# zhiyuns/REHRSeg

Measured on AMD Instinct MI355X. Metric: 3D patches/sec (fwd+bwd, 128^3 fp32), higher is better.
Workload: dtype f32; 1 GPU; FLAVR UNet_3D_3D(1,'unet_18',128,4) fwd+bwd+Adam, 1x1x128^3 patch per GPU, random-init weights; patches_per_gpu=1, global_batch=1, parallelism=dp1 (patch-parallel, flat-bucket RCCL all-reduce), wgrad_stream=True

## Files before the change

include/rehrseg_hip.h:

```cpp
#ifndef REHRSEG_HIP_H
#define REHRSEG_HIP_H

#include <stdint.h>

#ifdef __cplusplus
extern "C" {
#endif

#define REHR_OK 0
#define REHR_EINVAL -1
#define REHR_ENOSUP -2
#define REHR_EHIP -3

#define REHR_ACT_NONE 0
#define REHR_ACT_RELU 1
#define REHR_ACT_LRELU 2

typedef struct {
  int32_t count, off0, offs, k0, ks;
} rehr_axis_taps;

typedef struct {
  const float* x1;
  const float* x2;
// ... 3 lines not shown
  int32_t sd, sh, sw, bd, bh, bw;
  rehr_axis_taps td, th, tw;
  int32_t KH, KW;
  const float* wp;
  int32_t Npad;
  float* y;
  int32_t Dy, Hy, Wy, Cout, ldy;
  int32_t osd, osh, osw, obd, obh, obw;
  const float* bias;
  int32_t act;
  float slope;
  double* stats;
  int32_t stats_mode;
  int32_t tile_d, tile_h, tile_w;
  float* wino_ws;
  int64_t wino_ws_bytes;
  int32_t flags;
  int32_t debug_flags;
} rehr_gather_gemm_desc;

#define REHR_GG_Y_F32 1
#define REHR_GG_WS_READY 2
#define REHR_GG_WS_ONLY 4

#define REHR_DBG_GG_NO_HALO 1
#define REHR_DBG_GG_NO_FLAT8 2
#define REHR_DBG_GG_FLAT8_HALF 4
#define REHR_DBG_GG_FLAT8_FULL 8
#define REHR_DBG_GG_W32P_TWO_PER_CU 16
#define REHR_DBG_GG_W32P_ONE_PER_CU 32
#define REHR_DBG_GG_INTERLEAVE 64
#define REHR_DBG_GG_NO_TCONV_KS 128
#define REHR_DBG_GG_SLICE_MAJOR 256

int64_t rehr_gather_gemm_wino_bytes(const rehr_gather_gemm_desc* d);
#define REHR_GG_ROUTE_NONE 0
#define REHR_GG_ROUTE_FLAT8 1
#define REHR_GG_ROUTE_W32P 2
#define REHR_GG_ROUTE_BIG8 3
#define REHR_GG_ROUTE_SMALL 4
#define REHR_GG_ROUTE_FLAT22 5
#define REHR_GG_ROUTE_REGION22 6
int rehr_gather_gemm_wino_route(const rehr_gather_gemm_desc* d);
#define REHR_GG_DIRECT_NONE 0
#define REHR_GG_DIRECT_GENERIC 1
#define REHR_GG_DIRECT_HALO 2
#define REHR_GG_DIRECT_TCONV_KS 3
int rehr_gather_gemm_direct_route(const rehr_gather_gemm_desc* descs, int32_t count, int32_t bf16, int32_t* routes);
int rehr_gather_gemm_f32(const rehr_gather_gemm_desc* d, void* stream);
int rehr_gather_gemm_multi_f32(const rehr_gather_gemm_desc* descs, int32_t count,
                               void* stream);
int rehr_gather_gemm_wino_forms_f32(const rehr_gather_gemm_desc* descs, int32_t count, const float* w, int32_t D0,
                                    int32_t D1, int32_t T, int32_t dest_dim, int32_t dest_lo, int32_t src_lo,
                                    void* stream);
int rehr_gather_gemm_bf16(const rehr_gather_gemm_desc* d, void* stream);
int rehr_gather_gemm_multi_bf16(const rehr_gather_gemm_desc* descs, int32_t count, void* stream);
int rehr_pack_weights_bf16(const float* in, void* out, int32_t A, int32_t Apad, int32_t B, int32_t T,
                           int32_t transpose_ab, void* stream);

int rehr_sum_slabs_bias_act_f32(const float* slabs, int32_t S, int64_t slab_stride,
                                const float* bias, float* y, int64_t rows, int32_t C,
                                int32_t act, float slope, void* stream);

int rehr_sum_slabs_stats_f32(const float* slabs, int32_t S, int64_t slab_stride, const float* bias,
                             float* y, int32_t N, int64_t SV, int32_t C, int32_t act, float slope,
                             double* stats, void* stream);

int rehr_sum_slabs_bias_act_bf16(const float* slabs, int32_t S, int64_t slab_stride, const float* bias, void* y,
                                 int64_t rows, int32_t C, int32_t act, float slope, void* stream);
int rehr_sum_slabs_stats_bf16(const float* slabs, int32_t S, int64_t slab_stride, const float* bias, void* y,
                              int32_t N, int64_t SV, int32_t C, int32_t act, float slope, double* stats,
                              void* stream);

typedef struct {
  const float* l;
  int32_t ldl, Ca;
// ... 357 lines not shown
```

rehrseg_amd/csrc/gather_gemm.hip:

```cpp
#include "common.h"
#include "halo_shared.h"
#include "wino_shared.h"

namespace {

constexpr int BK = 32;
constexpr int LDS_LD = 36;
constexpr int NTHREADS = 256;

template <int BM, int BN, int WGM, int WGN, int LDSBUF>
__device__ __forceinline__ void gather_gemm_body(const GGParams& p, const int nblocks, const int logical_in = -1) {
  constexpr int WTM = BM / WGM, WTN = BN / WGN;
  constexpr int FM = WTM / 32, FN = WTN / 32;
  constexpr int AROWS = BM / 32, BROWS = BN / 32;
  static_assert(WGM * WGN == 4, "4 waves");
  const rehr_gather_gemm_desc& d = p.d;

  extern __shared__ __attribute__((aligned(16))) float smem[];
  float* As = smem;
  float* Bs = smem + LDSBUF * BM * LDS_LD;
  int* row_out = (int*)(Bs + LDSBUF * BN * LDS_LD);

  const int tid = threadIdx.x;
  const int lane = tid & 63, wave = tid >> 6;
// ... 382 lines not shown
    const rehr_axis_taps* ax[3] = {&d.td, &d.th, &d.tw};
    const int ext[3] = {T / (d.KH * d.KW), d.KH, d.KW};
    for (int a = 0; a < 3; ++a) {
      const int64_t first = ax[a]->k0, last = (int64_t)ax[a]->k0 + (int64_t)ax[a]->ks * (ax[a]->count - 1);
      if (first < 0 || first >= ext[a] || last < 0 || last >= ext[a]) return REHR_EINVAL;
    }
  }
  if (route[0].kind == DIRECT_TCONV_KS) return REHR_ENOSUP;
  WinoRoute r[MAX_PHASES];
  WinoPlan plan{};
  const WinoRoute joint = wino_joint_route(descs, count, plan);
  for (int i = 0; i < count; ++i) {
    r[i] = joint ? joint : wino_part_route(descs[i], count, plan);
    if (r[i] == WINO_NONE) return REHR_ENOSUP;
  }
  WinoWeightSrc src;
  const int64_t s0 = (int64_t)D1 * T, s1 = T;
  src.sn = dest_dim == 0 ? s0 : s1;
  src.sc = dest_dim == 0 ? s1 : s0;
  src.w = w + dest_lo * src.sn + src_lo * src.sc;
  return wino_forms_launch(r, descs, count, src, (hipStream_t)stream);
}

extern "C" int64_t rehr_gather_gemm_wino_bytes(const rehr_gather_gemm_desc* dp) {
  WinoPlan plan{};
  if (dp == nullptr || validate(*dp) != REHR_OK || wino_route(*dp, plan) == WINO_NONE) return 0;
  return plan.bytes;
}

extern "C" int rehr_gather_gemm_wino_route(const rehr_gather_gemm_desc* dp) {
  WinoPlan plan{};
  if (dp == nullptr || validate(*dp) != REHR_OK) return REHR_GG_ROUTE_NONE;
  const WinoRoute r = wino_route(*dp, plan);
  return r == WINO_NONE ? REHR_GG_ROUTE_NONE : (int)r | (plan.variant << 8);
}

extern "C" int rehr_gather_gemm_direct_route(const rehr_gather_gemm_desc* descs, int32_t count, int32_t bf16,
                                             int32_t* routes) {
  DirectRoute route[MAX_PHASES];
  if (routes == nullptr) return REHR_EINVAL;
  const int rc = direct_route(descs, count, bf16 ? 2 : 4, route);
  if (rc != REHR_OK) return rc;
  for (int i = 0; i < count; ++i) routes[i] = route[i].kind | (route[i].variant << 8);
  return REHR_OK;
}

extern "C" int rehr_gather_gemm_f32(const rehr_gather_gemm_desc* dp, void* stream) {
  if (dp == nullptr) return REHR_EINVAL;
  return rehr_gather_gemm_multi_f32(dp, 1, stream);
}
```

rehrseg_amd/csrc/wino_conv.hip:

```cpp
#include "common.h"
#include "wino_shared.h"
#include <cstdlib>

namespace {

constexpr int TH = 4, TW = 8;
constexpr int PH = 2 * TH + 2, PW = 2 * TW + 2;
constexpr int PVOX = PH * PW;
constexpr int LDX = 36;
constexpr int NX = (PVOX * 8 + 255) / 256;

struct WinoParams {
  rehr_gather_gemm_desc d;
  int nb_h, nb_w;
  int band_major;
  int kchunks;
  int dh0, dw0;
  const float* up;
  uint32_t up_bytes;
  int nsplit;
  rehr_axis_taps s_td[8];
  const float* s_up[8];
  uint32_t s_up_bytes[8];
  float* s_y[8];
// ... 188 lines not shown
#pragma unroll
    for (int q = 0; q < 16; ++q) t[rr][q] = ex[((rr * 2 + co) * 16 + q) * 64 + lane];
#pragma unroll
  for (int q = 0; q < 16; ++q) {
    const float yv = k0 * t[0][q] + t[1][q] + k2 * t[2][q] + k3 * t[3][q] + bv;
    const float v = fmaxf(yv, 0.f) + neg_slope * fminf(yv, 0.f);
    const int tile = (q & 3) + 8 * (q >> 2) + 4 * half;
    const int oh = oh0 + 2 * (tile / TW) + ro, ow = ow0 + 2 * (tile % TW) + co;
    const bool ok = colok & (oh < d.Lh) & (ow < d.Lw);
    if (ok) d.y[((((int64_t)n_img * d.Dy + od) * d.Hy + oh) * d.Wy + ow) * d.ldy + col_n] = v;
    s1_ += ok ? v : 0.f;
    s2_ += ok ? v * v : 0.f;
  }
  if (d.stats_mode != 0) {
    s1_ += __shfl_xor(s1_, 32, 64);
    s2_ += __shfl_xor(s2_, 32, 64);
    __syncthreads();
    float* red = smem;
    if (half == 0) {
      red[(r * 2 + 0) * 32 + col] = s1_;
      red[(r * 2 + 1) * 32 + col] = s2_;
    }
    __syncthreads();
    if (r == 0 && half == 0 && colok) {
      const float a1 = red[col] + red[64 + col] + red[128 + col] + red[192 + col];
      const float a2 = red[32 + col] + red[96 + col] + red[160 + col] + red[224 + col];
      double* st = d.stats + ((int64_t)n_img * d.Cout + col_n) * 2;
      atomicAdd(st, (double)a1);
      if (d.stats_mode == 2) atomicAdd(st + 1, (double)a2);
    }
  }
}

constexpr int PW2 = 18, PVOX2 = 18 * 18;
constexpr int RP2 = PW2 * LDX + 8;
constexpr int BUF2 = PW2 * RP2;

__global__ void wino_weights_frag_kernel(const rehr_gather_gemm_desc d, float* __restrict__ up, int kchunks) {
  const int cpad = kchunks * 32;
  const int64_t per = (int64_t)d.Npad * cpad;
  const int64_t per_src = (int64_t)d.Npad * d.Cin;
  const int64_t total = (int64_t)d.td.count * per;
  const int NT = d.Npad / 32;
  for (int64_t i = (int64_t)blockIdx.x * blockDim.x + threadIdx.x; i < total; i += (int64_t)gridDim.x * blockDim.x) {
    const int jd = (int)(i / per);
    const int64_t rem = i - (int64_t)jd * per;
    const int n = (int)(rem / cpad), ci = (int)(rem - (int64_t)n * cpad);
    float g[3][3];
#pragma unroll
    for (int jh = 0; jh < 3; ++jh)
#pragma unroll
      for (int jw = 0; jw < 3; ++jw) {
        const int a = d.bh + d.th.off0 + d.th.offs * jh + 1;
        const int b = d.bw + d.tw.off0 + d.tw.offs * jw + 1;
        const int wt = ((d.td.k0 + d.td.ks * jd) * d.KH + (d.th.k0 + d.th.ks * jh)) * d.KW + (d.tw.k0 + d.tw.ks * jw);
        const float v = ci < d.Cin ? d.wp[(int64_t)wt * per_src + (int64_t)n * d.Cin + ci] : 0.f;
#pragma unroll
        for (int aa = 0; aa < 3; ++aa)
#pragma unroll
          for (int bb = 0; bb < 3; ++bb)
            if (aa == a && bb == b) g[aa][bb] = v;
      }
    float u[16];
    wino_u33(g, u);
    const int nt = n >> 5, col = n & 31, chunk = ci >> 5, kk = (ci >> 3) & 3, half = (ci >> 2) & 1, e = ci & 3;
#pragma unroll
    for (int xi = 0; xi < 16; ++xi) {
      const int64_t o = (((((int64_t)jd * 16 + xi) * NT + nt) * kchunks + chunk) * 4 + kk) * 256 + (half * 32 + col) * 4 + e;
      up[o] = u[xi];
    }
  }
}

constexpr int NX8 = (PVOX2 * 8 + 511) / 512;

__global__ __launch_bounds__(512) void wino_conv_big8_kernel(const WinoParams p) {
  const rehr_gather_gemm_desc& d = p.d;
  extern __shared__ __attribute__((aligned(16))) float smem[];
  float* Xs = smem;
  constexpr int BUF = BUF2;

  const int tid = threadIdx.x, lane = tid & 63;
  const int wv = __builtin_amdgcn_readfirstlane(tid >> 6);
  const int r = wv & 3, fm = wv >> 2;
  const int half = lane >> 5, col = lane & 31;
  const int part = (p.nsplit > 1) ? (int)(blockIdx.z % p.nsplit) : 0;
  const int n_img = (p.nsplit > 1) ? (int)(blockIdx.z / p.nsplit) : (int)blockIdx.z;
  const rehr_axis_taps td = (p.nsplit > 1) ? p.s_td[part] : p.d.td;
  const float* const up = (p.nsplit > 1) ? p.s_up[part] : p.up;
  const uint32_t up_bytes = (p.nsplit > 1) ? p.s_up_bytes[part] : p.up_bytes;
  float* const yout = (p.nsplit > 1) ? p.s_y[part] : p.d.y;
  const int nt0 = blockIdx.y * 2, n0 = blockIdx.y * 64;
  int b = xcd_remap(blockIdx.x, gridDim.x);
  const int bw_ = b % p.nb_w; b /= p.nb_w;
  const int bh_ = p.band_major ? b / p.d.Ld : b % p.nb_h;
  const int od = p.band_major ? b % p.d.Ld : b / p.nb_h;
  const int oh0 = bh_ * 16, ow0 = bw_ * 16;

  const int i1 = (r == 0) ? 0 : 1, i2 = (r == 3) ? 3 : 2;
  const float s2 = (r == 1) ? 1.f : -1.f;
  const float rsign = (r == 2) ? -1.f : 1.f;
  const int th_ = fm * 4 + (col >> 3), tw_ = col & 7;
  const float* xa = Xs + (2 * th_ + i1) * RP2 + tw_ * LDX + 4 * half;
  const float* xb = Xs + (2 * th_ + i2) * RP2 + tw_ * LDX + 4 * half;

  int pvx[NX8];
  uint32_t pok = 0;
#pragma unroll
  for (int i = 0; i < NX8; ++i) {
    const int piece = tid + 512 * i;
    const int v = piece >> 3;
    const int ph = v / PW2, slot = v - ph * PW2;
    const int pw_ = slot < 9 ? 2 * slot : 2 * (slot - 9) + 1;
    const int ih = oh0 + p.dh0 + ph, iw = ow0 + p.dw0 + pw_;
    const bool ok = (piece < PVOX2 * 8) & ((unsigned)ih < (unsigned)d.Hi) & ((unsigned)iw < (unsigned)d.Wi);
    pvx[i] = ok ? ih * d.Wi + iw : 0;
    pok |= (ok ? 1u : 0u) << i;
  }
  const int pq = tid & 7;
  const uint32_t img_elems = (uint32_t)d.Di * d.Hi * d.Wi;
  constexpr int NXH = NX8 / 2;
  f32x4 rx[NXH];
  int jd_lo = td.count, jd_hi = -1;
  for (int j = 0; j < td.count; ++j) {
    const int id = od + d.bd + td.off0 + td.offs * j;
    if ((unsigned)id < (unsigned)d.Di) { jd_lo = min(jd_lo, j); jd_hi = max(jd_hi, j); }
  }
  const int items = p.kchunks * max(0, jd_hi - jd_lo + 1);
  struct Item { int chunk, jd; };
  auto advance = [&](Item& t) {
    if (++t.jd > jd_hi) { t.jd = jd_lo; ++t.chunk; }
  };
  auto fetch_to = [&](f32x4 (&rx)[NXH], const Item& t, const int lo) {
    const bool live = (t.chunk < p.kchunks) & (items > 0);
    const int jd = t.jd;
    const int cc = (live ? t.chunk : 0) * 32;
    const int id = od + d.bd + td.off0 + td.offs * jd;
    const bool first = cc < d.c1;
    const float* src = first ? d.x1 : d.x2;
    const uint32_t ld = (uint32_t)(first ? d.ldx1 : d.ldx2);
    const int coff = first ? cc : cc - d.c1;
    const uint32_t nrec = img_elems * ld * 4u;
    const __amdgpu_buffer_rsrc_t rs = __builtin_amdgcn_make_buffer_rsrc(
        const_cast<float*>(src) + (int64_t)n_img * img_elems * ld, 0, nrec, 0x00020000);
    const bool dok = live & ((unsigned)id < (unsigned)d.Di) & ((cc + pq * 4) < d.Cin);
    const uint32_t base = (uint32_t)(id * d.Hi * d.Wi) * ld * 4u + (uint32_t)(coff + pq * 4) * 4u;
#pragma unroll
    for (int i = 0; i < NXH; ++i) {
      const bool ok = dok & ((pok >> (lo + i)) & 1u);
      const uint32_t off = base + (uint32_t)pvx[lo + i] * ld * 4u;
      rx[i] = __builtin_bit_cast(f32x4, __builtin_amdgcn_raw_buffer_load_b128(rs, ok ? off : nrec, 0, 0));
    }
  };
  auto stage_from = [&](const f32x4 (&rx)[NXH], int buf, const int lo) {
#pragma unroll
    for (int i = 0; i < NXH; ++i) {
      const int piece = tid + 512 * (lo + i);
      const int v = piece >> 3, row = (v * 3641) >> 16;
      if (piece < PVOX2 * 8) *reinterpret_cast<f32x4*>(Xs + buf + v * LDX + row * 8 + pq * 4) = rx[i];
    }
  };
  auto fetch = [&](const Item& t, const int lo) { fetch_to(rx, t, lo); };
  auto stage = [&](int buf, const int lo) { stage_from(rx, buf, lo); };

  const __amdgpu_buffer_rsrc_t rsu =
      __builtin_amdgcn_make_buffer_rsrc(const_cast<float*>(up), 0, up_bytes, 0x00020000);
  const int NT = d.Npad / 32;
  const uint32_t xi_stride = (uint32_t)NT * p.kchunks * 4096u, nt_stride = (uint32_t)p.kchunks * 4096u;
  const uint32_t ulane = (uint32_t)lane * 16u;
  const uint32_t ubase = (uint32_t)(r * 4) * xi_stride + (uint32_t)nt0 * nt_stride;
  auto load_u = [&](const Item& t, const int kk, const int fn, f32x4 (&ub)[4]) {
    const int chunk = t.chunk < p.kchunks ? t.chunk : 0;
    const uint32_t base = ubase + (uint32_t)(t.jd * 16) * xi_stride + (uint32_t)(chunk * 4 + kk) * 1024u + fn * nt_stride;
#pragma unroll
    for (int c = 0; c < 4; ++c)
      ub[c] = __builtin_bit_cast(f32x4, __builtin_amdgcn_raw_buffer_load_b128(rsu, ulane, base + c * xi_stride, 0));
  };

  f32x16 acc[2][4];
#pragma unroll
  for (int fn = 0; fn < 2; ++fn)
#pragma unroll
    for (int c = 0; c < 4; ++c)
#pragma unroll
      for (int q = 0; q < 16; ++q) acc[fn][c][q] = 0.f;

  f32x4 ra[4], rb[4];
  auto issue_reads = [&](int buf, const int kk) {
#pragma unroll
    for (int j = 0; j < 4; ++j) {
// ... 72 lines not shown
  for (int it = 0; it < items; ++it) {
    const int cur = (it & 1) * BUF, nxt = cur ^ BUF;
    advance(ni);
    BIG8_PRIO(2);
    BIG8_KGROUP(0, VA, VB, ci, 1, issue_reads(cur, 1), fetch(ni, 0), (void)0)
    BIG8_PRIO(1);
    BIG8_KGROUP(1, VB, VA, ci, 2, issue_reads(cur, 2), (void)0, stage(nxt, 0))
    BIG8_KGROUP(2, VA, VB, ci, 3, issue_reads(cur, 3), fetch(ni, NXH), (void)0)
    __builtin_amdgcn_sched_barrier(0);
    BIG8_PRIO(0);
    stage(nxt, NXH);
    mfmas(0, VB, u0);
    __builtin_amdgcn_sched_barrier(0);
    load_u(ni, 0, 0, u0);
#ifdef BIG8_STAMPS
    const long long sa_ = __builtin_readcyclecounter();
#endif
    __syncthreads();
#ifdef BIG8_STAMPS
    b8_bar += __builtin_readcyclecounter() - sa_;
#endif
    __builtin_amdgcn_sched_barrier(0);
    BIG8_PRIO(3);
    issue_reads(nxt, 0);
    mfmas(1, VB, u1);
    combine(VA);
    __builtin_amdgcn_sched_barrier(0);
    load_u(ni, 0, 1, u1);
    ci = ni;
  }
#undef BIG8_KGROUP
  BIG8_PRIO(0);
#ifdef BIG8_STAMPS
  if ((threadIdx.x & 63) == 0 && blockIdx.x == 777 && blockIdx.y == 0 && blockIdx.z == 0)
    printf("big8 wave %d items %d: loop %lld cycles, barrier waits %lld\n", (int)(threadIdx.x >> 6), items,
           (long long)(__builtin_readcyclecounter() - b8_t0), b8_bar);
#endif
  __syncthreads();

  float* ex = smem;
#pragma unroll
  for (int fn = 0; fn < 2; ++fn) {
    const f32x16 T0 = (acc[fn][0] + acc[fn][1] - acc[fn][2]) * rsign;
    const f32x16 T1 = (acc[fn][1] + acc[fn][2] - acc[fn][3]) * rsign;
    float* e0 = ex + (((fm * 2 + fn) * 4 + r) * 2) * 16 * 64 + lane;
#pragma unroll
    for (int q = 0; q < 16; ++q) {
      e0[q * 64] = T0[q];
      e0[(16 + q) * 64] = T1[q];
    }
  }
  __syncthreads();
  const int ro = r >> 1, co = r & 1;
  const float k0 = ro == 0 ? 1.f : 0.f, k2 = ro == 0 ? 1.f : -1.f, k3 = ro == 0 ? 0.f : -1.f;
  const float neg_slope = d.act == REHR_ACT_NONE ? 1.f : (d.act == REHR_ACT_RELU ? 0.f : d.slope);
  float ssum[2][2];
  float* ybase = yout + ((((int64_t)n_img * d.Dy + od) * d.Hy + (oh0 + ro)) * d.Wy + (ow0 + co + 8 * half)) * d.ldy +
                 n0 + col;
  const int64_t rowstep = 2 * (int64_t)d.Wy * d.ldy, colstep = 2 * (int64_t)d.ldy;
  const bool interior = (oh0 + 16 <= d.Lh) & (ow0 + 16 <= d.Lw) & (n0 + 64 <= d.Cout);
#pragma unroll
  for (int fn = 0; fn < 2; ++fn) {
    const int col_n = n0 + fn * 32 + col;
    const bool colok = col_n < d.Cout;
    const float bv = (d.bias != nullptr && colok) ? d.bias[col_n] : 0.f;
    float s1_ = 0.f, s2_ = 0.f;
    const float* e0 = ex + ((fm * 2 + fn) * 4 * 2 + co) * 16 * 64 + lane;
    float t[4][16];
#pragma unroll
    for (int rr = 0; rr < 4; ++rr)
#pragma unroll
      for (int q = 0; q < 16; ++q) t[rr][q] = e0[(rr * 32 + q) * 64];
    float v[16];
#pragma unroll
    for (int q = 0; q < 16; ++q) {
      const float yv = k0 * t[0][q] + t[1][q] + k2 * t[2][q] + k3 * t[3][q] + bv;
      v[q] = fmaxf(yv, 0.f) + neg_slope * fminf(yv, 0.f);
    }
    float* yb = ybase + fn * 32 + (fm * 4) * rowstep;
    if (interior) {
#pragma unroll
      for (int q = 0; q < 16; ++q) {
        yb[(q >> 2) * rowstep + (q & 3) * colstep] = v[q];
        s1_ += v[q];
        s2_ += v[q] * v[q];
      }
    } else {
#pragma unroll
      for (int q = 0; q < 16; ++q) {
        const int oh = oh0 + 2 * (fm * 4 + (q >> 2)) + ro, ow = ow0 + 2 * ((q & 3) + 4 * half) + co;
        const bool ok = colok & (oh < d.Lh) & (ow < d.Lw);
        if (ok) yb[(q >> 2) * rowstep + (q & 3) * colstep] = v[q];
        s1_ += ok ? v[q] : 0.f;
        s2_ += ok ? v[q] * v[q] : 0.f;
      }
    }
    ssum[fn][0] = s1_ + __shfl_xor(s1_, 32, 64);
    ssum[fn][1] = s2_ + __shfl_xor(s2_, 32, 64);
  }
  if (d.stats_mode != 0) {
    __syncthreads();
    float* red = smem;
    if (half == 0) {
#pragma unroll
      for (int fn = 0; fn < 2; ++fn) {
        red[((wv * 2 + fn) * 2 + 0) * 32 + col] = ssum[fn][0];
        red[((wv * 2 + fn) * 2 + 1) * 32 + col] = ssum[fn][1];
      }
    }
    __syncthreads();
    if (wv < 2 && half == 0) {
      const int fn = wv, col_n = n0 + fn * 32 + col;
      if (col_n < d.Cout) {
        float a1 = 0.f, a2 = 0.f;
#pragma unroll
        for (int w = 0; w < 8; ++w) {
          a1 += red[((w * 2 + fn) * 2 + 0) * 32 + col];
          a2 += red[((w * 2 + fn) * 2 + 1) * 32 + col];
        }
        double* st = d.stats + ((int64_t)n_img * d.Cout + col_n) * 2;
        atomicAdd(st, (double)a1);
        if (d.stats_mode == 2) atomicAdd(st + 1, (double)a2);
      }
    }
  }
}

constexpr int W3_LD = 20, W3_RP = PW2 * W3_LD + 8;
template <int NFM> struct W3 {
  static constexpr int ROWS = 8 * NFM + 2, BUF = ROWS * W3_RP, VOX = ROWS * PW2, NTHR = 256 * NFM;
  static constexpr int NXT = (VOX * 4 + NTHR - 1) / NTHR;
};

template <int G>
__global__ __launch_bounds__(256 * G, G == 1 ? 2 : 1) void wino_conv_w32p_kernel(const WinoParams p) {
  constexpr int NTHR = 256 * G, VOX = W3<2 * G>::VOX, BUF = W3<2 * G>::BUF + 32;
  constexpr int W3P_NX = (VOX * 4 + NTHR - 1) / NTHR;
  const rehr_gather_gemm_desc& d = p.d;
  extern __shared__ __attribute__((aligned(16))) float smem[];
  float* Xs = smem;

  const int tid = threadIdx.x, lane = tid & 63;
  const int wv = __builtin_amdgcn_readfirstlane(tid >> 6);
  const int r = wv & 3, g = wv >> 2;
  const int half = lane >> 5, col = lane & 31;
  const int n_img = blockIdx.z;
  const int nt0 = blockIdx.y, n0 = blockIdx.y * 32;
  int b = xcd_remap(blockIdx.x, gridDim.x);
  const int bw_ = b % p.nb_w; b /= p.nb_w;
  const int bh_ = p.band_major ? b / p.d.Ld : b % p.nb_h;
  const int od = p.band_major ? b % p.d.Ld : b / p.nb_h;
  const int oh0 = bh_ * (16 * G), ow0 = bw_ * 16;

  const int i1 = (r == 0) ? 0 : 1, i2 = (r == 3) ? 3 : 2;
  const float s2 = (r == 1) ? 1.f : -1.f;
  const float rsign = (r == 2) ? -1.f : 1.f;
  const int th_ = g * 8 + (col >> 3), tw_ = col & 7;
  const float* xa = Xs + (2 * th_ + i1) * W3_RP + tw_ * W3_LD + 4 * half;
// ... 215 lines not shown
      for (int q = 0; q < 16; ++q) {
        const int oh = oh0 + 2 * (fm * 4 + (q >> 2)) + ro, ow = ow0 + 2 * ((q & 3) + 4 * half) + co;
        const bool ok = colok & (oh < d.Lh) & (ow < d.Lw);
        if (ok) yb[(q >> 2) * rowstep + (q & 3) * colstep] = v[q];
        s1_ += ok ? (double)v[q] : 0.0;
        s2_ += ok ? (double)v[q] * (double)v[q] : 0.0;
      }
    }
  }
  if (d.stats_mode != 0) {
    s1_ += __shfl_xor(s1_, 32, 64);
    s2_ += __shfl_xor(s2_, 32, 64);
    __syncthreads();
    double* red = reinterpret_cast<double*>(smem);
    if (half == 0) {
      red[(wv * 2 + 0) * 32 + col] = s1_;
      red[(wv * 2 + 1) * 32 + col] = s2_;
    }
    __syncthreads();
    if (wv == 0 && half == 0 && colok) {
      double a1 = 0.0, a2 = 0.0;
#pragma unroll
      for (int w = 0; w < 4 * G; ++w) {
        a1 += red[(w * 2 + 0) * 32 + col];
        a2 += red[(w * 2 + 1) * 32 + col];
      }
      double* st = d.stats + ((int64_t)n_img * d.Cout + col_n) * 2;
      atomicAdd(st, a1);
      if (d.stats_mode == 2) atomicAdd(st + 1, a2);
    }
  }
}

bool regions16_ok(const rehr_gather_gemm_desc& d) {
  if (d.Lh < 16 || d.Lw < 16) return false;
  const int64_t nb_h = (d.Lh + 15) / 16, nb_w = (d.Lw + 15) / 16;
  return nb_h * 16 * nb_w * 16 * 10 <= (int64_t)d.Lh * d.Lw * 13;
}
int w32_groups(const rehr_gather_gemm_desc& d) {
  const int64_t nb_h = (d.Lh + 31) / 32, nb_w = (d.Lw + 15) / 16;
  if (d.Lh >= 32 && nb_h * 32 * nb_w * 16 * 10 <= (int64_t)d.Lh * d.Lw * 13) return 4;
  return 2;
}

template <int G>
int launch_w32p(const WinoParams& p, hipStream_t stream) {
  constexpr size_t smem_x = (size_t)2 * (W3<2 * G>::BUF + 32) * sizeof(float);
  constexpr size_t smem_e = (size_t)2 * G * 4 * 2 * 16 * 64 * sizeof(float);
  constexpr size_t smem = smem_x > smem_e ? smem_x : smem_e;
  const int rc = set_dyn_lds_once<wino_conv_w32p_kernel<G>>((int)smem);
  if (rc != REHR_OK) return rc;
  dim3 grid((unsigned)((int64_t)p.nb_h * p.nb_w * p.d.Ld), p.d.Npad / 32, p.d.N);
  hipLaunchKernelGGL(wino_conv_w32p_kernel<G>, grid, dim3(256 * G), smem, stream, p);
  return REHR_OK;
}

}

WinoRoute wino_region_plan(const rehr_gather_gemm_desc& d, WinoPlan& plan) {
  if (d.sd != 1 || d.sh != 1 || d.sw != 1) return WINO_NONE;
  if (d.osd != 1 || d.osh != 1 || d.osw != 1 || d.obd || d.obh || d.obw) return WINO_NONE;
  if (d.Ld != d.Dy || d.Lh != d.Hy || d.Lw != d.Wy) return WINO_NONE;
  if (!three_taps(d.th, d.bh) || !three_taps(d.tw, d.bw)) return WINO_NONE;
  if (d.td.count < 1 || d.td.count > 256) return WINO_NONE;
  if (d.Lh < 8 || d.Lw < 8) return WINO_NONE;
  const WinoRoute r = !regions16_ok(d) ? WINO_SMALL : d.Npad % 64 ? WINO_W32P : WINO_BIG8;
  const int64_t nb_h = (d.Lh + 2 * TH - 1) / (2 * TH), nb_w = (d.Lw + 2 * TW - 1) / (2 * TW);
  if (r == WINO_SMALL && nb_h * 2 * TH * nb_w * 2 * TW * 100 > (int64_t)d.Lh * d.Lw * 134) return WINO_NONE;
  plan.bytes = wino_scratch_bytes(d, 16);
  if (plan.bytes == 0) return WINO_NONE;
  if (!gg_src_fits(d, (int64_t)d.Di * d.Hi * d.Wi, 4)) return WINO_NONE;
  if (nb_h * nb_w * d.Ld >= (1ll << 31) || d.Npad / 32 > 65535 || d.N > 65535) return WINO_NONE;
  plan.kchunks = (d.Cin + 31) / 32;
  plan.variant = 0;
  plan.nb_h = r == WINO_SMALL ? (int)nb_h : (d.Lh + 15) / 16;
  plan.nb_w = r == WINO_SMALL ? (int)nb_w : (d.Lw + 15) / 16;
  if (r == WINO_W32P) {
    const bool two = (d.debug_flags & REHR_DBG_GG_W32P_TWO_PER_CU) ? true
                     : (d.debug_flags & REHR_DBG_GG_W32P_ONE_PER_CU) ? false : d.Cin * d.td.count <= 96;
    plan.variant = (w32_groups(d) == 4 && !two) ? 2 : 1;
    plan.nb_h = (d.Lh + 16 * plan.variant - 1) / (16 * plan.variant);
  }
  return r;
}

bool wino_split_plan(const rehr_gather_gemm_desc* ds, int count, WinoPlan& plan) {
  if (count < 2 || count > 8 || (int64_t)ds[0].N * count > 65535) return false;
  if (wino_region_plan(ds[0], plan) != WINO_BIG8) return false;
  for (int i = 0; i < count; ++i) {
    const rehr_gather_gemm_desc& d = ds[i];
    WinoPlan q{};
    if (wino_region_plan(d, q) == WINO_NONE || !wino_ws_ok(d, q.bytes)) return false;
    if (d.bias || d.stats_mode || d.act != REHR_ACT_NONE || !gg_same_layer(d, ds[0], SAME_HW_TAPS)) return false;
  }
  return true;
}

int wino_weights_launch(WinoRoute r, const rehr_gather_gemm_desc& d, const WinoPlan& plan, hipStream_t stream) {
  if (r == WINO_SMALL)
    return wino_transform_launch<wino_weights_kernel>(d, (int64_t)d.td.count * d.Npad * d.Cin, 4096, stream);
  return wino_transform_launch<wino_weights_frag_kernel>(d, (int64_t)d.td.count * d.Npad * plan.kchunks * 32, 8192, stream,
                                                         plan.kchunks);
}

int wino_region_launch(WinoRoute r, const rehr_gather_gemm_desc* ds, int count, const WinoPlan& plan, hipStream_t stream) {
  const rehr_gather_gemm_desc& d = ds[0];
  WinoParams p;
  p.d = d;
  p.kchunks = plan.kchunks;
  p.dh0 = -1;
  p.dw0 = -1;
  p.nb_h = plan.nb_h;
  p.nb_w = plan.nb_w;
  p.band_major = (d.debug_flags & REHR_DBG_GG_SLICE_MAJOR) ? 0 : 1;
  p.nsplit = count > 1 ? count : 0;
  p.up = count > 1 ? nullptr : d.wino_ws;
  p.up_bytes = count > 1 ? 0 : (uint32_t)plan.bytes;
  for (int i = 0; count > 1 && i < count; ++i) {
    p.s_td[i] = ds[i].td;
    p.s_up[i] = ds[i].wino_ws;
    p.s_up_bytes[i] = (uint32_t)wino_scratch_bytes(ds[i], 16);
    p.s_y[i] = ds[i].y;
  }
  if (r == WINO_W32P) {
    const int rc = plan.variant == 2 ? launch_w32p<2>(p, stream) : launch_w32p<1>(p, stream);
    if (rc != REHR_OK) return rc;
  } else if (r == WINO_BIG8) {
    constexpr size_t smem_x = (size_t)2 * BUF2 * sizeof(float), smem_e = (size_t)4 * 4 * 2 * 16 * 64 * sizeof(float);
    constexpr size_t smem = smem_x > smem_e ? smem_x : smem_e;
    const int rc = set_dyn_lds_once<wino_conv_big8_kernel>((int)smem);
    if (rc != REHR_OK) return rc;
    dim3 grid((unsigned)((int64_t)p.nb_h * p.nb_w * d.Ld), d.Npad / 64, d.N * count);
    hipLaunchKernelGGL(wino_conv_big8_kernel, grid, dim3(512), smem, stream, p);
  } else {
    constexpr size_t smem_x = (size_t)2 * PVOX * LDX * sizeof(float), smem_e = (size_t)4 * 2 * 16 * 64 * sizeof(float);
    constexpr size_t smem = smem_x > smem_e ? smem_x : smem_e;
    static_assert(smem <= 64 * 1024, "wino_conv_kernel: dynamic LDS beyond the default limit");
    dim3 grid((unsigned)((int64_t)p.nb_h * p.nb_w * d.Ld), d.Npad / 32, d.N);
    hipLaunchKernelGGL(wino_conv_kernel, grid, dim3(256), smem, stream, p);
  }
  REHR_LAUNCH_CHECK();
  return REHR_OK;
}
```

rehrseg_amd/hip_backend.py:

```python
from __future__ import annotations

import ctypes as C
import os
import functools
import weakref

import torch
from torch.optim.optimizer import register_optimizer_step_post_hook as _register_step_hook

from . import lib as L

name = "hip"


def _stream():
    return C.c_void_p(torch.cuda.current_stream().cuda_stream)


_prof = None


def profile_start():
    global _prof
    _prof = []
# ... 255 lines not shown
    return _LazyPanel(w, A, Apad, B, T, transpose, part)


def _onepass_forms(arr, n, needs, lazy):
    global onepass_form_calls
    if not all(needs) or any(arr[i].Cout != lazy.A or arr[i].Cin != lazy.B for i in range(n)):
        return None
    w = lazy.w
    keep = _attach_ws(arr, n, needs, None, w)
    dest_dim = 1 if lazy.transpose else 0
    dest_lo = src_lo = 0
    if lazy.part is not None:
        if lazy.part[0] == dest_dim:
            dest_lo = lazy.part[1]
        else:
            src_lo = lazy.part[1]
    rc = L.load().rehr_gather_gemm_wino_forms_f32(arr, n, _ptr(w), w.shape[0], w.shape[1], lazy.T, dest_dim, dest_lo,
                                                  src_lo, _stream())
    if rc == -2:
        return keep, False
    L.check(rc, "rehr_gather_gemm_wino_forms_f32")
    for i in range(n):
        arr[i].flags |= L.GG_WS_READY
    onepass_form_calls += 1
    return keep, True


USE_WINOGRAD = True
USE_WINOGRAD_WGRAD = True
USE_HALO_BF16 = True
WGRAD_TAP_COLOCATE = True
USE_WGRAD_TAP_SKIP = True
W32P_BLOCKS = 0
PHASE_INTERLEAVE = False
WINO_BAND_MAJOR = True
USE_TCONV_KS = True
USE_WINO_FLAT8 = True
WINO_FLAT8_TILES = 0
wino_wgrad_launches = 0
wino_launches = 0


def _gg_desc(d, x1, x2, c1, src_dims, Cin, lattice, s, b, taps, KH, KW, wp, Npad, y, y_dims, Cout,
             os_, ob, bias, act, slope, stats, stats_mode, tile):
    _chk_dev(x1, x2, wp, y, bias, f64=(stats,))
    d.x1, d.x2, d.c1 = _ptr(x1), _ptr(x2), c1
    d.ldx1 = x1.shape[1]
    d.ldx2 = x2.shape[1] if x2 is not None else 0
    d.N = x1.shape[0]
    d.Di, d.Hi, d.Wi = src_dims
    d.Cin = Cin
    d.Ld, d.Lh, d.Lw = lattice
    d.sd, d.sh, d.sw = s
    d.bd, d.bh, d.bw = b
    d.td, d.th, d.tw = _taps(taps[0]), _taps(taps[1]), _taps(taps[2])
    d.KH, d.KW = KH, KW
    d.wp, d.Npad = _ptr(wp), Npad
    d.y = _ptr(y)
    d.Dy, d.Hy, d.Wy = y_dims
    d.Cout, d.ldy = Cout, y.shape[1]
    d.osd, d.osh, d.osw = os_
    d.obd, d.obh, d.obw = ob
    d.bias, d.act, d.slope = _ptr(bias), act, slope
    d.stats, d.stats_mode = _ptr(stats), stats_mode
    d.tile_d, d.tile_h, d.tile_w = tile
    d.wino_ws, d.wino_ws_bytes = None, 0
    d.flags = 0
    d.debug_flags = 0
    need = 0
    if x1.dtype == torch.bfloat16:
        if wp.dtype != torch.bfloat16 or (x2 is not None and x2.dtype != torch.bfloat16):
            raise L.RehrsegHipError("mixed-precision gather-GEMM: x1, x2 and the packed weights must all be bfloat16")
        if bias is not None and bias.dtype != torch.float32:
            raise L.RehrsegHipError("bias stays float32")
        d.flags = L.GG_Y_F32 if y.dtype == torch.float32 else 0
        d.debug_flags = (0 if USE_HALO_BF16 else L.DBG_GG_NO_HALO)
    elif wp.dtype != torch.float32 or y.dtype != torch.float32 or (x2 is not None and x2.dtype != torch.float32):
        raise L.RehrsegHipError("fp32 gather-GEMM: every operand must be float32")
    elif USE_WINOGRAD and tile[0] >= 0:
        d.debug_flags = ((0 if USE_WINO_FLAT8 else L.DBG_GG_NO_FLAT8) |
                         {1: L.DBG_GG_W32P_TWO_PER_CU, 2: L.DBG_GG_W32P_ONE_PER_CU}.get(W32P_BLOCKS, 0) |
                         {1: L.DBG_GG_FLAT8_HALF, 2: L.DBG_GG_FLAT8_FULL}.get(WINO_FLAT8_TILES, 0))
        need = L.load().rehr_gather_gemm_wino_bytes(C.byref(d))
    if PHASE_INTERLEAVE:
        d.debug_flags |= L.DBG_GG_INTERLEAVE
    if not USE_TCONV_KS:
        d.debug_flags |= L.DBG_GG_NO_TCONV_KS
    if not WINO_BAND_MAJOR:
        d.debug_flags |= L.DBG_GG_SLICE_MAJOR
    _gg_desc.need = need
    _gg_desc.sig = (c1, x1.shape[1], x2.shape[1] if x2 is not None else 0, x1.shape[0], tuple(src_dims), Cin,
                    tuple(lattice), tuple(s), tuple(b), tuple(tuple(t) for t in taps), KH, KW, Npad, tuple(y_dims), Cout,
                    y.shape[1], tuple(os_), tuple(ob), bias is not None, act, stats_mode, tuple(tile), d.debug_flags)
    return _algo_flops(d.N, lattice, s, b, taps, src_dims, Cin, Cout) if _prof is not None else 0.0


def _attach_ws(descs, n, needs, sigs, wp):
    if not any(needs):
        return None
    global wino_launches
    wino_launches += sum(1 for nb in needs if nb)
    dev = wp.device
    pf = _form_of_panel.get(id(wp)) if WEIGHT_FORM_CACHE else None
    p = pf.param() if pf is not None else None
    if p is None or not _keeps_forms(p):
        keeps = [torch.empty(nb // 4, dtype=torch.float32, device=dev) if nb else None for nb in needs]
        for i in range(n):
            if needs[i]:
                descs[i].wino_ws, descs[i].wino_ws_bytes = _ptr(keeps[i]), needs[i]
        return keeps
    key = ("ws", id(p), id(pf), tuple(sigs))
    f = _forms.get(key)
    if f is None or f.param() is not p or f.dep is not pf:
        outs = [torch.empty(nb // 4, dtype=torch.float32, device=dev) if nb else None for nb in needs]
# ... 28 lines not shown


def _gg_tag(arr, n=1, bf16=False):
    d = arr[0]
    name = _ROUTE_NAMES.get(wino_route(d)[0]) if d.wino_ws else None
    if name is None:
        try:
            kinds = [_DIRECT_NAMES[bf16].get(r, "none") for r in direct_route(arr, n, bf16)]
            name = "+".join(sorted(set(kinds), key=kinds.index))
        except L.RehrsegHipError:
            name = "invalid"
    return (f"N{d.N} {d.Cin}->{d.Cout} lattice {d.Ld}x{d.Lh}x{d.Lw} stride {d.sd}{d.sh}{d.sw} "
            f"taps {d.td.count}x{d.th.count}x{d.tw.count}" + (" +x2" if d.x2 else "") + f" [{name}]")


_ROUTE_NAMES = {L.GG_ROUTE_FLAT8: "flat8", L.GG_ROUTE_W32P: "w32p", L.GG_ROUTE_BIG8: "big8", L.GG_ROUTE_SMALL: "small",
                L.GG_ROUTE_FLAT22: "flat22", L.GG_ROUTE_REGION22: "region22"}
_DIRECT_NAMES = {False: {(L.GG_DIRECT_GENERIC, 0): "generic", (L.GG_DIRECT_TCONV_KS, 0): "tconv_ks",
                         (L.GG_DIRECT_HALO, 1): "halo bn64", (L.GG_DIRECT_HALO, 2): "halo bn32"},
                 True: {(L.GG_DIRECT_GENERIC, 0): "generic", (L.GG_DIRECT_TCONV_KS, 0): "tconv_ks",
                        (L.GG_DIRECT_HALO, 1): "halo 4x8x16", (L.GG_DIRECT_HALO, 2): "halo 8x8x8",
                        (L.GG_DIRECT_HALO, 3): "halo 2x16x16"}}


def direct_route(descs, count, bf16):
    out = (C.c_int32 * count)()
    L.check(L.load().rehr_gather_gemm_direct_route(descs, count, int(bool(bf16)), out), "rehr_gather_gemm_direct_route")
    return [(r & 255, (r >> 8) & 255) for r in out]


def wino_route(d):
    r = int(L.load().rehr_gather_gemm_wino_route(C.byref(d)))
    return r & 255, (r >> 8) & 255


def _gg_family(d):
    if _prof is None:
        return None
    if not d.wino_ws:
        return "gather_gemm"
    route = wino_route(d)[0]
    if route == L.GG_ROUTE_NONE:
        return "gather_gemm"
    return "wino22_conv" if route in (L.GG_ROUTE_FLAT22, L.GG_ROUTE_REGION22) else "wino_conv"


def _with_wp(args, wp):
    return args[:11] + (wp,) + args[12:]


def _set_panel(arr, n, panel):
    for i in range(n):
        arr[i].wp = _ptr(panel)


def gather_gemm(*args):
    lazy = args[11] if isinstance(args[11], _LazyPanel) else None
    if lazy is not None:
        args = _with_wp(args, lazy.w)
    d = L.GatherGemmDesc()
    flops = _gg_desc(d, *args)
    if args[0].dtype == torch.bfloat16:
        with _timed("gather_gemm_bf16", flops, lambda: _gg_tag((L.GatherGemmDesc * 1)(d), bf16=True)):
            L.check(L.load().rehr_gather_gemm_bf16(C.byref(d), _stream()), "rehr_gather_gemm_bf16")
        return
    arr = (L.GatherGemmDesc * 1)(d)
# ... 1213 lines not shown
```

rehrseg_amd/lib.py:

```python
from __future__ import annotations

import ctypes as C
import os
import re
from typing import Optional

_HERE = os.path.dirname(os.path.abspath(__file__))
LIB_PATH = os.environ.get("REHRSEG_HIP_LIB") or os.path.join(_HERE, "librehrseg_hip.so")
HEADER_PATH = os.path.join(os.path.dirname(_HERE), "include", "rehrseg_hip.h")

ACT_NONE, ACT_RELU, ACT_LRELU = 0, 1, 2
ABI_VERSION = 6
GG_Y_F32 = 1
GG_WS_READY = 2
GG_WS_ONLY = 4
DBG_WGRAD_DIRECT = 1
DBG_WGRAD_NO_TAP_SKIP = 2
DBG_WGRAD_NO_TAP_COLOCATE = 4
DBG_GG_NO_HALO = 1
DBG_GG_NO_FLAT8 = 2
DBG_GG_FLAT8_HALF = 4
DBG_GG_FLAT8_FULL = 8
DBG_GG_W32P_TWO_PER_CU = 16
DBG_GG_W32P_ONE_PER_CU = 32
DBG_GG_INTERLEAVE = 64
DBG_GG_NO_TCONV_KS = 128
DBG_GG_SLICE_MAJOR = 256
GG_ROUTE_NONE, GG_ROUTE_FLAT8, GG_ROUTE_W32P, GG_ROUTE_BIG8 = 0, 1, 2, 3
GG_ROUTE_SMALL, GG_ROUTE_FLAT22, GG_ROUTE_REGION22 = 4, 5, 6
GG_DIRECT_NONE, GG_DIRECT_GENERIC, GG_DIRECT_HALO, GG_DIRECT_TCONV_KS = 0, 1, 2, 3

_i32, _i64, _f32 = C.c_int32, C.c_int64, C.c_float
_vp = C.c_void_p


class AxisTaps(C.Structure):
    _fields_ = [("count", _i32), ("off0", _i32), ("offs", _i32), ("k0", _i32), ("ks", _i32)]

    def __init__(self, count=1, off0=0, offs=1, k0=0, ks=1):
        super().__init__(count, off0, offs, k0, ks)

    def astuple(self):
        return (self.count, self.off0, self.offs, self.k0, self.ks)


class GatherGemmDesc(C.Structure):
    _fields_ = [
        ("x1", _vp), ("x2", _vp), ("c1", _i32), ("ldx1", _i32), ("ldx2", _i32),
        ("N", _i32), ("Di", _i32), ("Hi", _i32), ("Wi", _i32), ("Cin", _i32),
        ("Ld", _i32), ("Lh", _i32), ("Lw", _i32),
        ("sd", _i32), ("sh", _i32), ("sw", _i32), ("bd", _i32), ("bh", _i32), ("bw", _i32),
        ("td", AxisTaps), ("th", AxisTaps), ("tw", AxisTaps), ("KH", _i32), ("KW", _i32),
        ("wp", _vp), ("Npad", _i32),
        ("y", _vp), ("Dy", _i32), ("Hy", _i32), ("Wy", _i32), ("Cout", _i32), ("ldy", _i32),
        ("osd", _i32), ("osh", _i32), ("osw", _i32), ("obd", _i32), ("obh", _i32), ("obw", _i32),
        ("bias", _vp), ("act", _i32), ("slope", _f32),
        ("stats", _vp), ("stats_mode", _i32),
        ("tile_d", _i32), ("tile_h", _i32), ("tile_w", _i32),
        ("wino_ws", _vp), ("wino_ws_bytes", _i64),
        ("flags", _i32), ("debug_flags", _i32),
# ... 26 lines not shown
        ("act", _i32), ("slope", _f32), ("stats", _vp), ("stats_mode", _i32),
    ]


PATCH_F32, PATCH_U8, PATCH_MAX_ITEMS = 0, 1, 16


class PatchItem(C.Structure):
    _fields_ = [("src", _vp), ("base", _i64), ("stride", _i64 * 4), ("lo", _i32 * 4), ("hi", _i32 * 4)]


class PatchGatherDesc(C.Structure):
    _fields_ = [("n_items", _i32), ("dims", _i32 * 4), ("src_dtype", _i32), ("scale", _f32), ("bias", _f32),
                ("dst", _vp), ("dst_item_stride", _i64)]


DS_MAX_LEVELS = 8


class SegDsLevel(C.Structure):
    _fields_ = [("logits", _vp), ("target", _vp), ("unc", _vp), ("dlogits", _vp), ("S", _i64),
                ("d", _i32), ("h", _i32), ("w", _i32), ("ld", _i32), ("ldd", _i32), ("weight", _f32)]


class PyramidLevel(C.Structure):
    _fields_ = [("dst", _vp), ("d", _i32), ("h", _i32), ("w", _i32), ("iz", _vp), ("iy", _vp), ("ix", _vp)]


_P_GG, _P_WG, _P_DC =C.POINTER(GatherGemmDesc), C.POINTER(WgradDesc), C.POINTER(DirectConvDesc)

PROTOTYPES = {
    "rehr_gather_gemm_wino_bytes": (_i64, [_P_GG]),
    "rehr_gather_gemm_wino_route": (C.c_int, [_P_GG]),
    "rehr_gather_gemm_direct_route": (C.c_int, [_P_GG, _i32, _i32, C.POINTER(_i32)]),
    "rehr_gather_gemm_f32": (C.c_int, [_P_GG, _vp]),
    "rehr_gather_gemm_multi_f32": (C.c_int, [_P_GG, _i32, _vp]),
    "rehr_gather_gemm_wino_forms_f32": (C.c_int, [_P_GG, _i32, _vp, _i32, _i32, _i32, _i32, _i32, _i32, _vp]),
    "rehr_gather_gemm_bf16": (C.c_int, [_P_GG, _vp]),
    "rehr_gather_gemm_multi_bf16": (C.c_int, [_P_GG, _i32, _vp]),
    "rehr_pack_weights_bf16": (C.c_int, [_vp, _vp, _i32, _i32, _i32, _i32, _i32, _vp]),
    "rehr_sum_slabs_bias_act_f32": (C.c_int, [_vp, _i32, _i64, _vp, _vp, _i64, _i32, _i32, _f32, _vp]),
    "rehr_sum_slabs_stats_f32": (C.c_int, [_vp, _i32, _i64, _vp, _vp, _i32, _i64, _i32, _i32, _f32, _vp, _vp]),
    "rehr_sum_slabs_bias_act_bf16": (C.c_int, [_vp, _i32, _i64, _vp, _vp, _i64, _i32, _i32, _f32, _vp]),
    "rehr_sum_slabs_stats_bf16": (C.c_int, [_vp, _i32, _i64, _vp, _vp, _i32, _i64, _i32, _i32, _f32, _vp, _vp]),
    "rehr_wgrad_workspace_bytes": (_i64, [_P_WG]),
    "rehr_wgrad_uses_winograd": (C.c_int, [_P_WG]),
    "rehr_wgrad_f32": (C.c_int, [_P_WG, _vp]),
    "rehr_wgrad_bf16_workspace_bytes": (_i64, [_P_WG]),
    "rehr_wgrad_bf16": (C.c_int, [_P_WG, _vp]),
    "rehr_pack_weights_f32": (C.c_int, [_vp, _vp, _i32, _i32, _i32, _i32, _i32, _vp]),
    "rehr_conv_small_cin_fwd_f32": (C.c_int, [_P_DC, _vp]),
    "rehr_im2col_f32": (C.c_int, [_P_DC, _vp, _i32, _vp]),
    "rehr_conv_small_cin_wgrad_workspace_bytes": (_i64, [_P_DC]),
    "rehr_conv_small_cin_wgrad_on_mfma": (C.c_int, [_P_DC]),
    "rehr_conv_small_cin_fwd_on_mfma": (C.c_int, [_P_DC]),
    "rehr_conv_small_cin_fwd_ybf16": (C.c_int, [_P_DC, _vp]),
    "rehr_conv_small_cin_wgrad_dybf16": (C.c_int, [_P_DC, _vp, _vp, _vp, _i64, _vp]),
    "rehr_conv_small_cin_wgrad_f32": (C.c_int, [_P_DC, _vp, _vp, _vp, _i64, _vp]),
    "rehr_conv_small_cout_fwd_f32": (C.c_int, [_P_DC, _vp]),
    "rehr_conv_small_cout_dgrad_f32": (C.c_int, [_P_DC, _vp, _vp]),
    "rehr_conv_small_cout_wgrad_workspace_bytes": (_i64, [_P_DC]),
    "rehr_conv_small_cout_wgrad_f32": (C.c_int, [_P_DC, _vp, _vp, _vp, _i64, _vp]),
    "rehr_se_gate_fwd_f32": (C.c_int, [_vp, _vp, _vp, _vp, _vp, _i32, _i32, _i64, _vp]),
    "rehr_scale_res_act_fwd_f32": (C.c_int, [_vp, _i32, _vp, _vp, _i32, _vp, _i32, _i32, _i64, _i32, _i32, _f32, _vp]),
    "rehr_scale_res_act_bwd_f32": (C.c_int, [_vp, _i32, _vp, _i32, _vp, _i32, _vp, _vp, _i32, _vp, _i32, _vp,
                                             _i32, _i64, _i32, _i32, _f32, _vp]),
# ... 144 lines not shown
```

Measured before the change: 17.01 patches/s.

## Add half-region big8 Winograd variant running two 256-thread blocks per CU

Templates the big8 Winograd conv kernel on the number of frame rows (NFM). It adds a 256-thread, half-height variant with launch bounds allowing two blocks per CU, and doubles the grid accordingly. The half variant is chosen when kchunks times live depth taps is small, so short-K layers get more blocks and better latency hiding instead of leaving 512-thread blocks underfilled. The trade-off is more halo rows per output and extra redundant input staging. Debug flags and a query entry point allow forcing either variant.

Result: no change. 17.01 patches/s, median of 3 (-0.0%).

```diff
diff --git a/include/rehrseg_hip.h b/include/rehrseg_hip.h
--- a/include/rehrseg_hip.h
+++ b/include/rehrseg_hip.h
@@ -59,6 +59,8 @@
 #define REHR_DBG_GG_INTERLEAVE 64
 #define REHR_DBG_GG_NO_TCONV_KS 128
 #define REHR_DBG_GG_SLICE_MAJOR 256
+#define REHR_DBG_GG_BIG8_TWO_PER_CU 512
+#define REHR_DBG_GG_BIG8_ONE_PER_CU 1024
 
 int64_t rehr_gather_gemm_wino_bytes(const rehr_gather_gemm_desc* d);
 #define REHR_GG_ROUTE_NONE 0
@@ -69,6 +71,7 @@
 #define REHR_GG_ROUTE_FLAT22 5
 #define REHR_GG_ROUTE_REGION22 6
 int rehr_gather_gemm_wino_route(const rehr_gather_gemm_desc* d);
+int rehr_gather_gemm_wino_big8_blocks(const rehr_gather_gemm_desc* d);
 #define REHR_GG_DIRECT_NONE 0
 #define REHR_GG_DIRECT_GENERIC 1
 #define REHR_GG_DIRECT_HALO 2
diff --git a/rehrseg_amd/csrc/gather_gemm.hip b/rehrseg_amd/csrc/gather_gemm.hip
--- a/rehrseg_amd/csrc/gather_gemm.hip
+++ b/rehrseg_amd/csrc/gather_gemm.hip
@@ -438,7 +438,13 @@
   WinoPlan plan{};
   if (dp == nullptr || validate(*dp) != REHR_OK) return REHR_GG_ROUTE_NONE;
   const WinoRoute r = wino_route(*dp, plan);
-  return r == WINO_NONE ? REHR_GG_ROUTE_NONE : (int)r | (plan.variant << 8);
+  return r == WINO_NONE ? REHR_GG_ROUTE_NONE : (int)r | ((r == WINO_BIG8 ? 0 : plan.variant) << 8);
+}
+
+extern "C" int rehr_gather_gemm_wino_big8_blocks(const rehr_gather_gemm_desc* dp) {
+  WinoPlan plan{};
+  if (dp == nullptr || validate(*dp) != REHR_OK) return 0;
+  return wino_route(*dp, plan) == WINO_BIG8 ? plan.variant : 0;
 }
 
 extern "C" int rehr_gather_gemm_direct_route(const rehr_gather_gemm_desc* descs, int32_t count, int32_t bf16,
diff --git a/rehrseg_amd/csrc/wino_conv.hip b/rehrseg_amd/csrc/wino_conv.hip
--- a/rehrseg_amd/csrc/wino_conv.hip
+++ b/rehrseg_amd/csrc/wino_conv.hip
@@ -244,9 +244,15 @@
   }
 }
 
-constexpr int PW2 = 18, PVOX2 = 18 * 18;
+constexpr int PW2 = 18;
 constexpr int RP2 = PW2 * LDX + 8;
-constexpr int BUF2 = PW2 * RP2;
+template <int NFM> struct B8 {
+  static constexpr int ROWS = 8 * NFM + 2, VOX = ROWS * PW2, BUF = ROWS * RP2, NTHR = 256 * NFM;
+  static constexpr int NX = (VOX * 8 + NTHR - 1) / NTHR;
+  static constexpr size_t SMEM_X = (size_t)2 * BUF * sizeof(float);
+  static constexpr size_t SMEM_E = (size_t)NFM * 2 * 4 * 2 * 16 * 64 * sizeof(float);
+  static constexpr size_t SMEM = SMEM_X > SMEM_E ? SMEM_X : SMEM_E;
+};
 
 __global__ void wino_weights_frag_kernel(const rehr_gather_gemm_desc d, float* __restrict__ up, int kchunks) {
   const int cpad = kchunks * 32;
@@ -284,17 +290,19 @@
   }
 }
 
-constexpr int NX8 = (PVOX2 * 8 + 511) / 512;
-
-__global__ __launch_bounds__(512) void wino_conv_big8_kernel(const WinoParams p) {
+template <int NFM>
+__global__ __launch_bounds__(256 * NFM, NFM == 1 ? 2 : 1) void wino_conv_big8_kernel(const WinoParams p) {
+  constexpr int NTHR = B8<NFM>::NTHR, PVOX2 = B8<NFM>::VOX, BUF = B8<NFM>::BUF, NX8 = B8<NFM>::NX;
   const rehr_gather_gemm_desc& d = p.d;
   extern __shared__ __attribute__((aligned(16))) float smem[];
   float* Xs = smem;
-  constexpr int BUF = BUF2;
+#ifdef BIG8_STAMPS
+  const long long b8_k0 = __builtin_readcyclecounter();
+#endif
 
   const int tid = threadIdx.x, lane = tid & 63;
   const int wv = __builtin_amdgcn_readfirstlane(tid >> 6);
-  const int r = wv & 3, fm = wv >> 2;
+  const int r = wv & 3, fm = NFM == 2 ? wv >> 2 : 0;
   const int half = lane >> 5, col = lane & 31;
   const int part = (p.nsplit > 1) ? (int)(blockIdx.z % p.nsplit) : 0;
   const int n_img = (p.nsplit > 1) ? (int)(blockIdx.z / p.nsplit) : (int)blockIdx.z;
@@ -304,10 +312,13 @@
   float* const yout = (p.nsplit > 1) ? p.s_y[part] : p.d.y;
   const int nt0 = blockIdx.y * 2, n0 = blockIdx.y * 64;
   int b = xcd_remap(blockIdx.x, gridDim.x);
+  const int hf = NFM == 1 ? b & 1 : 0;
+  if (NFM == 1) b >>= 1;
   const int bw_ = b % p.nb_w; b /= p.nb_w;
   const int bh_ = p.band_major ? b / p.d.Ld : b % p.nb_h;
   const int od = p.band_major ? b % p.d.Ld : b / p.nb_h;
-  const int oh0 = bh_ * 16, ow0 = bw_ * 16;
+  const int oh0 = bh_ * 16 + 8 * hf, ow0 = bw_ * 16;
+  if (NFM == 1 && oh0 >= d.Lh) return;
 
   const int i1 = (r == 0) ? 0 : 1, i2 = (r == 3) ? 3 : 2;
   const float s2 = (r == 1) ? 1.f : -1.f;
@@ -320,7 +331,7 @@
   uint32_t pok = 0;
 #pragma unroll
   for (int i = 0; i < NX8; ++i) {
-    const int piece = tid + 512 * i;
+    const int piece = tid + NTHR * i;
     const int v = piece >> 3;
     const int ph = v / PW2, slot = v - ph * PW2;
     const int pw_ = slot < 9 ? 2 * slot : 2 * (slot - 9) + 1;
@@ -367,7 +378,7 @@
   auto stage_from = [&](const f32x4 (&rx)[NXH], int buf, const int lo) {
 #pragma unroll
     for (int i = 0; i < NXH; ++i) {
-      const int piece = tid + 512 * (lo + i);
+      const int piece = tid + NTHR * (lo + i);
       const int v = piece >> 3, row = (v * 3641) >> 16;
       if (piece < PVOX2 * 8) *reinterpret_cast<f32x4*>(Xs + buf + v * LDX + row * 8 + pq * 4) = rx[i];
     }
@@ -506,9 +517,10 @@
 #undef BIG8_KGROUP
   BIG8_PRIO(0);
 #ifdef BIG8_STAMPS
+  const long long b8_t1 = __builtin_readcyclecounter();
   if ((threadIdx.x & 63) == 0 && blockIdx.x == 777 && blockIdx.y == 0 && blockIdx.z == 0)
     printf("big8 wave %d items %d: loop %lld cycles, barrier waits %lld\n", (int)(threadIdx.x >> 6), items,
-           (long long)(__builtin_readcyclecounter() - b8_t0), b8_bar);
+           (long long)(b8_t1 - b8_t0), b8_bar);
 #endif
   __syncthreads();
 
@@ -532,7 +544,7 @@
   float* ybase = yout + ((((int64_t)n_img * d.Dy + od) * d.Hy + (oh0 + ro)) * d.Wy + (ow0 + co + 8 * half)) * d.ldy +
                  n0 + col;
   const int64_t rowstep = 2 * (int64_t)d.Wy * d.ldy, colstep = 2 * (int64_t)d.ldy;
-  const bool interior = (oh0 + 16 <= d.Lh) & (ow0 + 16 <= d.Lw) & (n0 + 64 <= d.Cout);
+  const bool interior = (oh0 + 8 * NFM <= d.Lh) & (ow0 + 16 <= d.Lw) & (n0 + 64 <= d.Cout);
 #pragma unroll
   for (int fn = 0; fn < 2; ++fn) {
     const int col_n = n0 + fn * 32 + col;
@@ -588,7 +600,7 @@
       if (col_n < d.Cout) {
         float a1 = 0.f, a2 = 0.f;
 #pragma unroll
-        for (int w = 0; w < 8; ++w) {
+        for (int w = 0; w < 4 * NFM; ++w) {
           a1 += red[((w * 2 + fn) * 2 + 0) * 32 + col];
           a2 += red[((w * 2 + fn) * 2 + 1) * 32 + col];
         }
@@ -598,6 +610,14 @@
       }
     }
   }
+#ifdef BIG8_STAMPS
+  {
+    const unsigned hw = __builtin_amdgcn_s_getreg((31 << 11) | 4), xcc = __builtin_amdgcn_s_getreg((31 << 11) | 20) & 15u;
+    if (tid == 0 && blockIdx.y == 0 && blockIdx.z == 0 && xcc == 0 && ((hw >> 13) & 7u) == 0)
+      printf("big8<%d> block %d cu %u items %d: start %lld loop %lld .. %lld end %lld\n", NFM, (int)blockIdx.x,
+             (hw >> 8) & 31u, items, b8_k0, b8_t0, b8_t1, (long long)__builtin_readcyclecounter());
+  }
+#endif
 }
 
 constexpr int W3_LD = 20, W3_RP = PW2 * W3_LD + 8;
@@ -879,6 +899,8 @@
   }
 }
 
+constexpr int BIG8_HALF_MAX_ITEMS = 6;
+
 bool regions16_ok(const rehr_gather_gemm_desc& d) {
   if (d.Lh < 16 || d.Lw < 16) return false;
   const int64_t nb_h = (d.Lh + 15) / 16, nb_w = (d.Lw + 15) / 16;
@@ -888,6 +910,16 @@
   const int64_t nb_h = (d.Lh + 31) / 32, nb_w = (d.Lw + 15) / 16;
   if (d.Lh >= 32 && nb_h * 32 * nb_w * 16 * 10 <= (int64_t)d.Lh * d.Lw * 13) return 4;
   return 2;
+}
+
+template <int NFM>
+int launch_big8(const WinoParams& p, int count, hipStream_t stream) {
+  static_assert(NFM == 2 || 2 * B8<NFM>::SMEM <= 160 * 1024, "two half-region blocks per CU");
+  const int rc = set_dyn_lds_once<wino_conv_big8_kernel<NFM>>((int)B8<NFM>::SMEM);
+  if (rc != REHR_OK) return rc;
+  dim3 grid((unsigned)((int64_t)p.nb_h * p.nb_w * p.d.Ld * (3 - NFM)), p.d.Npad / 64, p.d.N * count);
+  hipLaunchKernelGGL(wino_conv_big8_kernel<NFM>, grid, dim3(B8<NFM>::NTHR), B8<NFM>::SMEM, stream, p);
+  return REHR_OK;
 }
 
 template <int G>
@@ -928,6 +960,15 @@
     plan.variant = (w32_groups(d) == 4 && !two) ? 2 : 1;
     plan.nb_h = (d.Lh + 16 * plan.variant - 1) / (16 * plan.variant);
   }
+  if (r == WINO_BIG8) {
+    const int step = d.td.offs < 0 ? -d.td.offs : d.td.offs;
+    const int reach = step == 0 ? d.td.count : (d.Di + step - 1) / step;
+    const int live_taps = d.td.count < reach ? d.td.count : reach;
+    const bool half = (d.debug_flags & REHR_DBG_GG_BIG8_TWO_PER_CU) ? true
+                      : (d.debug_flags & REHR_DBG_GG_BIG8_ONE_PER_CU) ? false
+                                                                      : plan.kchunks * live_taps <= BIG8_HALF_MAX_ITEMS;
+    plan.variant = half && 2ll * plan.nb_h * plan.nb_w * d.Ld < (1ll << 31) ? 1 : 2;
+  }
   return r;
 }
 
@@ -973,12 +1014,8 @@
     const int rc = plan.variant == 2 ? launch_w32p<2>(p, stream) : launch_w32p<1>(p, stream);
     if (rc != REHR_OK) return rc;
   } else if (r == WINO_BIG8) {
-    constexpr size_t smem_x = (size_t)2 * BUF2 * sizeof(float), smem_e = (size_t)4 * 4 * 2 * 16 * 64 * sizeof(float);
-    constexpr size_t smem = smem_x > smem_e ? smem_x : smem_e;
-    const int rc = set_dyn_lds_once<wino_conv_big8_kernel>((int)smem);
+    const int rc = plan.variant == 1 ? launch_big8<1>(p, count, stream) : launch_big8<2>(p, count, stream);
     if (rc != REHR_OK) return rc;
-    dim3 grid((unsigned)((int64_t)p.nb_h * p.nb_w * d.Ld), d.Npad / 64, d.N * count);
-    hipLaunchKernelGGL(wino_conv_big8_kernel, grid, dim3(512), smem, stream, p);
   } else {
     constexpr size_t smem_x = (size_t)2 * PVOX * LDX * sizeof(float), smem_e = (size_t)4 * 2 * 16 * 64 * sizeof(float);
     constexpr size_t smem = smem_x > smem_e ? smem_x : smem_e;
diff --git a/rehrseg_amd/hip_backend.py b/rehrseg_amd/hip_backend.py
--- a/rehrseg_amd/hip_backend.py
+++ b/rehrseg_amd/hip_backend.py
@@ -311,6 +311,7 @@
 WGRAD_TAP_COLOCATE = True
 USE_WGRAD_TAP_SKIP = True
 W32P_BLOCKS = 0
+BIG8_BLOCKS = 0
 PHASE_INTERLEAVE = False
 WINO_BAND_MAJOR = True
 USE_TCONV_KS = True
@@ -359,6 +360,7 @@
     elif USE_WINOGRAD and tile[0] >= 0:
         d.debug_flags = ((0 if USE_WINO_FLAT8 else L.DBG_GG_NO_FLAT8) |
                          {1: L.DBG_GG_W32P_TWO_PER_CU, 2: L.DBG_GG_W32P_ONE_PER_CU}.get(W32P_BLOCKS, 0) |
+                         {1: L.DBG_GG_BIG8_TWO_PER_CU, 2: L.DBG_GG_BIG8_ONE_PER_CU}.get(BIG8_BLOCKS, 0) |
                          {1: L.DBG_GG_FLAT8_HALF, 2: L.DBG_GG_FLAT8_FULL}.get(WINO_FLAT8_TILES, 0))
         need = L.load().rehr_gather_gemm_wino_bytes(C.byref(d))
     if PHASE_INTERLEAVE:
@@ -453,6 +455,10 @@
 def wino_route(d):
     r = int(L.load().rehr_gather_gemm_wino_route(C.byref(d)))
     return r & 255, (r >> 8) & 255
+
+
+def wino_big8_blocks(d):
+    return int(L.load().rehr_gather_gemm_wino_big8_blocks(C.byref(d)))
 
 
 def _gg_family(d):
diff --git a/rehrseg_amd/lib.py b/rehrseg_amd/lib.py
--- a/rehrseg_amd/lib.py
+++ b/rehrseg_amd/lib.py
@@ -26,6 +26,8 @@
 DBG_GG_INTERLEAVE = 64
 DBG_GG_NO_TCONV_KS = 128
 DBG_GG_SLICE_MAJOR = 256
+DBG_GG_BIG8_TWO_PER_CU = 512
+DBG_GG_BIG8_ONE_PER_CU = 1024
 GG_ROUTE_NONE, GG_ROUTE_FLAT8, GG_ROUTE_W32P, GG_ROUTE_BIG8 = 0, 1, 2, 3
 GG_ROUTE_SMALL, GG_ROUTE_FLAT22, GG_ROUTE_REGION22 = 4, 5, 6
 GG_DIRECT_NONE, GG_DIRECT_GENERIC, GG_DIRECT_HALO, GG_DIRECT_TCONV_KS = 0, 1, 2, 3
@@ -118,6 +120,7 @@
 PROTOTYPES = {
     "rehr_gather_gemm_wino_bytes": (_i64, [_P_GG]),
     "rehr_gather_gemm_wino_route": (C.c_int, [_P_GG]),
+    "rehr_gather_gemm_wino_big8_blocks": (C.c_int, [_P_GG]),
     "rehr_gather_gemm_direct_route": (C.c_int, [_P_GG, _i32, _i32, C.POINTER(_i32)]),
     "rehr_gather_gemm_f32": (C.c_int, [_P_GG, _vp]),
     "rehr_gather_gemm_multi_f32": (C.c_int, [_P_GG, _i32, _vp]),
```
